# chlhnu/DOT-SOCP

Measured on AMD Instinct MI355X. Metric: ADMM iters/sec on NxNxT dot2d staggered grid at 1/2/4/8 MI355X, higher is better.
Workload: dtype f64

## Files before the change

dot-socp_amd/capi.py:

```python
import ctypes
import os

import numpy as np

_HERE = os.path.dirname(os.path.abspath(__file__))
LIB_PATH = os.path.join(_HERE, "lib", "libdotsocp.so")

i64 = ctypes.c_longlong
dbl = ctypes.c_double
vp = ctypes.c_void_p


class DotsocpError(RuntimeError):
    def __init__(self, code, msg):
        super().__init__(f"libdotsocp error {code}: {msg}")
        self.code = code


class Problem(ctypes.Structure):
    _fields_ = [("dim", ctypes.c_int), ("weighted", ctypes.c_int),
                ("ny", i64), ("nx", i64), ("nt", i64),
                ("D", dbl), ("E", dbl), ("cScale", dbl), ("dScale", dbl),
                ("normc", dbl), ("normd", dbl)]

# ... 30 lines not shown
    "dotsocp_bfd_conj1d": (ctypes.c_int, [vp, vp, i64, i64, dbl]),
    "dotsocp_oper_poisson": (ctypes.c_int, [vp, vp, i64, i64, i64, dbl]),
    "dotsocp_dctn": (ctypes.c_int, [vp, i64, i64, i64, ctypes.c_int]),
    "dotsocp_proj_soc_dev": (ctypes.c_int, [vp, vp, i64, i64, vp]),
    "dotsocp_bfd_dev": (ctypes.c_int, [vp, vp, i64, i64, i64, dbl, dbl, vp]),
    "dotsocp_bfd_conj_dev": (ctypes.c_int, [vp, vp, i64, i64, i64, dbl, vp]),
    "dotsocp_create": (vp, [ctypes.POINTER(Problem), ctypes.c_int, ctypes.c_int]),
    "dotsocp_create_multi": (vp, [ctypes.POINTER(Problem), ctypes.c_int, ctypes.c_int]),
    "dotsocp_destroy": (None, [vp]),
    "dotsocp_rccl_unique_id": (ctypes.c_int, [vp]),
    "dotsocp_attach_rccl": (ctypes.c_int, [vp, vp, ctypes.c_int, ctypes.c_int]),
    "dotsocp_slab_range": (ctypes.c_int, [i64, ctypes.c_int, ctypes.c_int, ctypes.POINTER(i64), ctypes.POINTER(i64)]),
    "dotsocp_field_len": (i64, [ctypes.POINTER(Problem), ctypes.c_int]),
    "dotsocp_dct_algorithm": (ctypes.c_int, [i64]),
    "dotsocp_tsolve_tri_safe": (ctypes.c_int, [i64, i64, i64]),
    "dotsocp_cone_writes_beta": (ctypes.c_int, [i64, dbl, i64, ctypes.c_int, ctypes.c_int, ctypes.c_int, dbl, dbl]),
    "dotsocp_rescale_due": (ctypes.c_int, [i64, ctypes.c_int, dbl, dbl]),
    "dotsocp_qcone_form": (ctypes.c_int, [i64, dbl, i64, ctypes.c_int, ctypes.c_int, ctypes.c_int, ctypes.c_int, dbl, dbl]),
    "dotsocp_release_cache": (i64, []),
    "dotsocp_upload": (ctypes.c_int, [vp, ctypes.c_int, vp]),
    "dotsocp_upload_layers": (ctypes.c_int, [vp, ctypes.c_int, vp, i64, i64]),
    "dotsocp_download": (ctypes.c_int, [vp, ctypes.c_int, vp]),
    "dotsocp_begin": (ctypes.c_int, [vp, ctypes.POINTER(Opts)]),
    "dotsocp_begin_method": (ctypes.c_int, [vp, ctypes.POINTER(Opts), ctypes.c_int, ctypes.POINTER(AccOpts)]),
    "dotsocp_run": (ctypes.c_int, [vp, i64, ctypes.POINTER(i64)]),
    "dotsocp_recover_outputs": (ctypes.c_int, [vp, vp, vp, vp, vp, vp, vp, vp, vp]),
    "dotsocp_jump_next_level": (ctypes.c_int, [vp, vp]),
    "dotsocp_finish": (ctypes.c_int, [vp, ctypes.POINTER(Result)]),
    "dotsocp_get_history": (ctypes.c_int, [vp, vp, vp, vp, vp]),
    "dotsocp_set_profiling": (ctypes.c_int, [vp, ctypes.c_int]),
# ... 76 lines not shown
```

dot-socp_amd/csrc/capi.hip:

```cpp
#include <cstring>
#include <new>

#include "comm.h"
#include "solver.h"

using namespace dotsocp;

namespace dotsocp {
extern thread_local std::string g_last_error;
int dotsocp_slab_range_impl(i64 nt, int world, int rank, i64 *t0, i64 *t1);
}

struct dotsocp_ctx {
    Solver s;
};

static int require_device() {
    int n = 0;
    if (hipGetDeviceCount(&n) != hipSuccess || n <= 0) {
        set_error("no HIP device available (libdotsocp has no CPU fallback)");
        return DOTSOCP_ENODEVICE;
    }
    return 0;
}
// ... 178 lines not shown
    DS_CHECK(pl.make(ny, nx, nt));
    const double pi = 3.14159265358979323846;
    auto table = [&](DevBuf &d, i64 m) -> int {
        std::vector<double> t((size_t)m);
        for (i64 k = 0; k < m; ++k) t[k] = (2.0 * (double)(m - 1) * (double)(m - 1)) * (1.0 - cos(pi * (double)k / (double)m));
        DS_CHECK(d.alloc(m));
        DS_HIP(hipMemcpy(d.p, t.data(), sizeof(double) * m, hipMemcpyHostToDevice));
        return 0;
    };
    DS_CHECK(table(cy, ny));
    DS_CHECK(table(cx, nx));
    DS_CHECK(table(ct, nt));
    DS_HIP(hipMemcpy(da.p, rhs, sizeof(double) * n, hipMemcpyHostToDevice));
    Grid g;
    g.set(ny, nx, nt, 0, nt);
    DS_CHECK(launch_dct_axis(pl.py, da.p, db.p, ny, nx, nt, 0, 0, nullptr));
    DS_CHECK(launch_dct_axis(pl.px, db.p, da.p, ny, nx, nt, 1, 0, nullptr));
    DS_CHECK(launch_poisson_t_single(pl.pt, g, kernelScale, cy.p, cx.p, ct.p, da.p, db.p, 0, nullptr, tsolve_tri_allowed()));
    DS_CHECK(launch_dct_axis(pl.px, da.p, db.p, ny, nx, nt, 1, 1, nullptr));
    DS_CHECK(launch_dct_axis(pl.py, db.p, da.p, ny, nx, nt, 0, 1, nullptr));
    DS_HIP(hipDeviceSynchronize());
    DS_HIP(hipMemcpy(res, da.p, sizeof(double) * n, hipMemcpyDeviceToHost));
    return 0;
}

dotsocp_ctx *dotsocp_create(const dotsocp_problem *prob, int device, int nslabs) {
    dotsocp_ctx *c = new (std::nothrow) dotsocp_ctx();
    if (!c) { set_error("out of host memory"); return nullptr; }
    if (c->s.init(prob, device, nslabs) != 0) {
        delete c;
        return nullptr;
    }
    return c;
}

// ... 26 lines not shown
}

int dotsocp_attach_rccl(dotsocp_ctx *ctx, const unsigned char id[128], int rank, int world) {
    if (!ctx) { set_error("ctx is NULL"); return DOTSOCP_EINVAL; }
    return ctx->s.attach_rccl(id, rank, world);
}

#define CTX_OR_FAIL()                                      \
    do {                                                   \
        if (!ctx) { set_error("ctx is NULL"); return DOTSOCP_EINVAL; } \
        (void)hipGetLastError();    \
    } while (0)

int dotsocp_dct_algorithm(dotsocp_i64 n) { return dct_choose_algorithm(n); }
int dotsocp_tsolve_tri_safe(dotsocp_i64 ny, dotsocp_i64 nx, dotsocp_i64 nt) { return tsolve_tri_safe(ny, nx, nt) ? 1 : 0; }

int dotsocp_cone_writes_beta(dotsocp_i64 it, double last_sigma_it, dotsocp_i64 maxit, int check_step_by_step,
                             int last_of_run, int rescale, double maxFeas, double relGap) {
    return cone_writes_beta(it, last_sigma_it, maxit, check_step_by_step != 0, last_of_run != 0, rescale, maxFeas, relGap) ? 1 : 0;
}
int dotsocp_rescale_due(dotsocp_i64 it, int rescale, double maxFeas, double relGap) {
    return rescale_due(it, rescale, maxFeas, relGap) ? 1 : 0;
}
int dotsocp_qcone_form(dotsocp_i64 it, double last_sigma_it, dotsocp_i64 maxit, int check_step_by_step, int last_of_run,
                       int next_last_of_run, int rescale, double maxFeas, double relGap) {
    return qcone_form(it, last_sigma_it, maxit, check_step_by_step != 0, last_of_run != 0, next_last_of_run != 0, rescale,
                      maxFeas, relGap);
}

dotsocp_i64 dotsocp_field_len(const dotsocp_problem *p, int field) {
// ... 94 lines not shown
```

dot-socp_amd/csrc/dct.hip:

```cpp
#include "cdft.h"
#include "dct_families.h"
#include "fft_lds.h"
#include "kernels.h"
#include "pfa.h"

#include <cstdlib>
#include <cstring>

namespace dotsocp {

#define CDFT_DEFAULT_MIN 500

int dct_choose_algorithm(i64 n) {
    static const bool pfa_on = !(getenv("DOTSOCP_PFA") && atoi(getenv("DOTSOCP_PFA")) == 0);
    static const bool cdft_on = !(getenv("DOTSOCP_CDFT") && atoi(getenv("DOTSOCP_CDFT")) == 0);
    static const i64 nb = [] {
        const char *e = getenv("DOTSOCP_CDFT_MIN");
        const i64 v = e ? atoll(e) : CDFT_DEFAULT_MIN;
        return v < 48 ? (i64)48 : v;
    }();
    if (n <= 1) return DCT_ALG_NONE;
    if ((n & (n - 1)) == 0) return DCT_ALG_FFT;
    if (pfa_supported(n)) return pfa_on ? DCT_ALG_PFA : DCT_ALG_DENSE;
    if (cdft_on && n == 257) return DCT_ALG_RADER;
// ... 164 lines not shown
    return !(e && strcmp(e, "dct") == 0);
}

int launch_poisson_t_single(const DctPlan *pt, const Grid &g, double kscale, const double *cy, const double *cx,
                            const double *ct, double *p, double *p2, i64 pitch0, hipStream_t st, bool allow_tri) {
    const i64 ny = g.ny, nx = g.nx, nt = g.nt;
    if (allow_tri && tsolve_tri_preferred(nt, dct_plan_is_pow2(pt), g.plane) && tsolve_tri_safe(ny, nx, nt))
        return launch_tsolve_tri(g, nt, kscale, cy, cx, p, st);
    if (dct_plan_has_tsolve(pt))
        return launch_dct_t_solve(pt, p, p, ny, ny * nx, 0, ny * nx, nt, kscale, cy, cx, ct, st, pitch0);
    DS_CHECK(launch_dct_axis(pt, p, p2, ny, nx, nt, 2, 0, st, pitch0));
    DS_CHECK(launch_spectral_divide(p2, ny, nt, 0, nx, kscale, cy, cx, ct, st, pitch0));
    return launch_dct_axis(pt, p2, p, ny, nx, nt, 2, 1, st, pitch0);
}

}
```

dot-socp_amd/csrc/dct_families.h:

```cpp
#pragma once
#include "common.h"

namespace dotsocp {

struct LineMap;
struct Pow2Plan;
struct DensePlan;

#define DCT_THREADS 256

Pow2Plan *pow2_plan_create(i64 n);
void pow2_plan_destroy(Pow2Plan *p);
int pow2_launch_axis0(const Pow2Plan *p, const double *src, double *dst, const LineMap &map, int inverse, hipStream_t st);
int pow2_launch_strided(const Pow2Plan *p, const double *src, double *dst, const LineMap &map, int inverse, hipStream_t st);
int pow2_launch_tsolve(const Pow2Plan *p, const double *src, double *dst, i64 ny, i64 nplane, i64 line0, i64 nl,
                       double kscale, const double *cy, const double *cx, const double *ct, hipStream_t st, i64 pitch0);

DensePlan *dense_plan_create(i64 n);
void dense_plan_destroy(DensePlan *p);
int dense_launch(const DensePlan *p, const double *src, double *dst, const LineMap &map, bool axis0, int inverse,
                 hipStream_t st);

}
```

dot-socp_amd/csrc/dct_pow2.hip:

```cpp
#include "dct_families.h"
#include "device_utils.h"
#include "fft_lds.h"
#include "kernels.h"

#include <cmath>
#include <cstdint>
#include <cstdlib>
#include <type_traits>
#include <utility>
#include <vector>

namespace dotsocp {

struct Pow2Plan {
    i64 n;
    int lg;
    double2 *tw;
    double2 *ww;
};

Pow2Plan *pow2_plan_create(i64 n) {
    Pow2Plan *p = new Pow2Plan();
    p->n = n;
    p->lg = 0;
// ... 556 lines not shown
                Bv = make_double2(p0.y, p1.y);
            } else {
                const double2 v0 = r[padi(bitrev(j0, LG))], v1 = r[padi(bitrev(n - 1 - j0, LG))];
                Av = make_double2(v0.x, v1.x);
                Bv = make_double2(v0.y, v1.y);
            }
            *(double2 *)(out + (2 * rr) * ls + 2 * j0) = Av;
            *(double2 *)(out + (2 * rr + 1) * ls + 2 * j0) = Bv;
        }
        if (tile + stride < nTiles) asm volatile("s_waitcnt vmcnt(%0)" ::"i"(PIPE_NS) : "memory");
        lds_barrier();
        if (tile + 2 * stride < nTiles) dma(tile + 2 * stride, b);
    }
}

template <int MODE , int LG>
__global__ void __launch_bounds__(PIPE_THREADS) k_dct_strided_pipe(const double *__restrict__ src, double *__restrict__ dst,
                                                                    LineMap map, int nTiles, const double2 *__restrict__ tw,
                                                                    const double2 *__restrict__ ww) {
    extern __shared__ double2 lds[];
    constexpr int n = 1 << LG;
    constexpr int lrows = PIPE_LG_CPLX - LG;
    constexpr int NP = 1 << lrows;
    constexpr int BUF = 1 << PIPE_LG_CPLX;
    constexpr bool BIG = LG > 10;
    constexpr int NTW = BIG ? (n >> 2) : (n >> 1), NWW = BIG ? (n >> 1) + 1 : n;
    double2 *twS = lds + 2 * BUF, *wwS = twS + NTW;
    const int tid = threadIdx.x, lane = tid & 63;
    const int wave = __builtin_amdgcn_readfirstlane(tid >> 6);
    for (int i = tid; i < NTW; i += PIPE_THREADS) twS[i] = tw[i];
// ... 429 lines not shown
        for_const<0, 1>(inverse ? 1 : 0, [&](auto i) {
            DS_KLAUNCH(k_dct_axis0_wg<decltype(i)::value != 0>, dim3(wblocks), dim3(DCT_WG_THREADS), lds, st, src, dst,
                       map.nLines, map.outerStride, lg, lrows, tw, ww);
        });
        DS_HIP(hipGetLastError());
        return 0;
    }
    for_const<0, 1>(inverse ? 1 : 0, [&](auto i) {
        DS_KLAUNCH(k_dct_axis0<decltype(i)::value != 0>, dim3(blocks), dim3(DCT_THREADS), lds, st, src, dst, map.nLines,
                   map.outerStride, lg, lrw, tw, ww);
    });
    DS_HIP(hipGetLastError());
    return 0;
}

}
```

dot-socp_amd/csrc/kernels.h:

```cpp
#pragma once
#include "common.h"
#include "defer.h"

namespace dotsocp {

struct LoopCoef {
    double s;
    double sf;
    double dF;
    double at, ax, ay;
    double tau;
    double c1, c2;
    double dinv1, dinv2;
};

enum {
    S_Q2 = 0, S_Z2, S_APHI2, S_ALPHA2, S_BETA2, S_FBBETA2, S_PRIM1, S_PRIM2, S_DUAL1, S_DUAL2,
    S_COMPLEM, S_DOTCOMP, S_RHO2, S_RHOFQ2, S_MRHOB, S_M2, S_RHOB2, S_QALPHA, S_CPHI, S_PHI2,
    S_COUNT
};

struct KktCoef {
    double sigma;
    double kappa;
// ... 153 lines not shown
    int world;
    i64 cut[DS_MAX_WORLD + 1];
};
int launch_pencil_pack(bool pack, const PencilCuts &pc, i64 plane, i64 ntl, double *slab, double *stage, hipStream_t st);

#define TRI_EXTRA 256
int launch_tri_local(const Grid &g, i64 nt, double kscale, const double *cy, const double *cx, const PencilCuts &pc,
                     const double *r, double *send, hipStream_t st);
int launch_tri_reduced(const Grid &g, i64 nt, double kscale, const double *cy, const double *cx, const PencilCuts &pc,
                       int rank, i64 l0, i64 nl, const i64 *slab_n, const double *recv, double *back, double *zero_work,
                       hipStream_t st, const double *own_recv = nullptr, double *own_back = nullptr);
int launch_tri_final(const Grid &g, i64 nt, double kscale, const double *cy, const double *cx, const PencilCuts &pc,
                     const double *back, double *x, hipStream_t st);
bool tsolve_tri_supported(i64 nt);
bool tsolve_tri_preferred(i64 nt, bool pow2, i64 plane);
bool tsolve_tri_safe(i64 ny, i64 nx, i64 nt);
int launch_tsolve_tri(const Grid &g, i64 nt, double kscale, const double *cy, const double *cx, double *x, hipStream_t st);
struct GatherMsgs {
    const double *src[DS_MAX_WORLD];
    double *dst[DS_MAX_WORLD];
    i64 count[DS_MAX_WORLD];
    int n;
};
int launch_gather_msgs(const GatherMsgs &m, hipStream_t st);

#define KKT_SLICES 64
struct KktWork {
    double *partials;
    i64 maxBlocks;
    double *sums;
// ... 26 lines not shown
void dct_plan_destroy(DctPlan *p);
int launch_dct_axis(const DctPlan *p, const double *src, double *dst, i64 n0, i64 n1, i64 n2, int axis,
                    int inverse, hipStream_t st, i64 pitch0 = 0);
bool dct_plan_is_pow2(const DctPlan *p);
bool dct_plan_has_tsolve(const DctPlan *p);
int launch_dct_t_solve(const DctPlan *p, const double *src, double *dst, i64 ny, i64 nplane, i64 line0, i64 nl,
                       i64 nt, double kscale, const double *cy, const double *cx, const double *ct, hipStream_t st,
                       i64 pitch0 = 0);
int launch_spectral_divide_pencil(double *data, i64 ny, i64 line0, i64 nl, i64 nt, double kscale, const double *cy,
                                  const double *cx, const double *ct, hipStream_t st);
int launch_spectral_divide(double *data, i64 ny, i64 nt, i64 x0, i64 nxl, double kscale, const double *cy,
                           const double *cx, const double *ct, hipStream_t st, i64 pitch0 = 0);
bool tsolve_tri_allowed();
int launch_poisson_t_single(const DctPlan *pt, const Grid &g, double kscale, const double *cy, const double *cx,
                            const double *ct, double *p, double *p2, i64 pitch0, hipStream_t st, bool allow_tri);

}
```

dot-socp_amd/csrc/solver.hip:

```cpp
#include "solver.h"

#include <algorithm>
#include <cmath>
#include <cstring>

#include "comm.h"

namespace dotsocp {

void Solver::update_coef() {
    lc.s = E / D;
    lc.sf = edge_factor(lc.s);
    lc.dF = E / dScale;
    const double ht = 1.0 / (double)(nt - 1);
    lc.at = D * (1.0 / ht);
    lc.ax = (nx > 1) ? D * (1.0 / (1.0 / (double)(nx - 1))) : 0.0;
    lc.ay = (ny > 1) ? D * (1.0 / (1.0 / (double)(ny - 1))) : 0.0;
    lc.tau = opts.tau;
    const double tmp = (E / D) * (E / D);
    if (prob.weighted) { lc.c1 = 2.0 * tmp; lc.c2 = tmp; }
    else { lc.c1 = 1.0 + 2.0 * tmp; lc.c2 = 1.0 + tmp; }
    lc.dinv1 = 1.0 / lc.c1;
    lc.dinv2 = 1.0 / lc.c2;
}
// ... 159 lines not shown
    if (canary_enabled() && getenv("DOTSOCP_CANARY_SELFTEST")) {
        Slab &s0 = slabs[0];
        DS_CHECK(use(s0));
        const double v = 1.0;
        DS_HIP(ds_memcpy_async(s0.c + s0.g.Nphi, &v, sizeof v, hipMemcpyHostToDevice, s0.st));
        DS_HIP(ds_stream_synchronize(s0.st));
    }
    begun = true;
    elapsed_prev = 0.0;
    elapsed_agreed = 0.0;
    t_begin = std::chrono::steady_clock::now();
    return 0;
}

int Solver::poisson_all(const PhiHooks *hooks) {
    const i64 plane = slabs[0].g.plane;
    const bool tp2 = dct_plan_has_tsolve(devres[0]->pt);
    FOR_SLABS(s) {
        const Grid &g = s.g;
        DS_CHECK(launch_dct_axis(s.res->py, s.w0, s.w1, g.ny, g.nx, g.ntl, 0, 0, s.st, g.py));
        DS_CHECK(launch_dct_axis(s.res->px, s.w1, s.w0, g.ny, g.nx, g.ntl, 1, 0, s.st, g.py));
    }
    bool tri = multi() && tri_tsolve && world <= DS_MAX_WORLD;
    for (auto &s : slabs) tri = tri && s.g.ntl <= TRI_EXTRA;
    if (tri) {
        DS_CHECK(poisson_t_tridiag(hooks));
    } else {
    if (hooks && hooks->fill) {
        prof_end(PH_POISSON);
        DS_CHECK(hooks->fill());
        prof_begin(PH_POISSON);
    }
    if (hooks && hooks->behind) DS_CHECK(hooks->behind());
    if (multi()) {
        prof_begin(PH_TRANSPOSE);
        DS_CHECK(transpose(true));
        prof_end(PH_TRANSPOSE);
    }
    FOR_SLABS(s) {
        double *p = multi() ? s.pencil : s.w0;
        double *p2 = multi() ? s.pencil2 : s.w1;
        if (!multi()) {
            DS_CHECK(launch_poisson_t_single(s.res->pt, s.g, D * D, s.res->cy, s.res->cx, s.res->ct, p, p2, s.g.py, s.st, tri_tsolve));
        } else if (tp2) {
            DS_CHECK(launch_dct_t_solve(s.res->pt, p, p, s.g.py, plane, s.l0, s.nl, nt, D * D, s.res->cy, s.res->cx, s.res->ct, s.st));
        } else {
            DS_CHECK(launch_dct_axis(s.res->pt, p, p2, s.nl, 1, nt, 2, 0, s.st));
            DS_CHECK(launch_spectral_divide_pencil(p2, s.g.py, s.l0, s.nl, nt, D * D, s.res->cy, s.res->cx, s.res->ct, s.st));
            DS_CHECK(launch_dct_axis(s.res->pt, p2, p, s.nl, 1, nt, 2, 1, s.st));
        }
    }
    if (multi()) {
        prof_begin(PH_TRANSPOSE);
        DS_CHECK(transpose(false));
        prof_end(PH_TRANSPOSE);
    }
    }
    FOR_SLABS(s) {
        const Grid &g = s.g;
        DS_CHECK(launch_dct_axis(s.res->px, s.w0, s.w1, g.ny, g.nx, g.ntl, 1, 1, s.st, g.py));
        DS_CHECK(launch_dct_axis(s.res->py, s.w1, s.phi, g.ny, g.nx, g.ntl, 0, 1, s.st, g.py));
    }
    return 0;
}

int Solver::poisson_phi() {
    if (begun) { set_error("poisson_phi() must precede begin()"); return DOTSOCP_ESTATE; }
    cur_dev = -1;
    DS_CHECK(use_dev(device));
    DS_CHECK(ensure_alloc());
    D = prob.D;
// ... 730 lines not shown
```

dot-socp_amd/csrc/tri.hip:

```cpp
#include "device_utils.h"
#include "kernels.h"

#include <cmath>
#include <cstdint>
#include <cstdlib>
#include <mutex>

namespace dotsocp {

struct TriGeom {
    i64 ny, plane, ntl;
    int first, last;
    double beta;
    double kscale;
    const double *cy, *cx;
    PencilCuts pc;
};

__device__ __forceinline__ double tri_aprime(const TriGeom &g, i64 m) { return (g.cy[m % g.ny] + g.cx[m / g.ny]) / g.beta; }

__device__ __forceinline__ int tri_owner(const PencilCuts &pc, i64 m, i64 plane) {
    int j = (int)((m * pc.world) / plane);
    while (j > 0 && m < pc.cut[j]) --j;
    while (j < pc.world - 1 && m >= pc.cut[j + 1]) ++j;
    return j;
}

__device__ __forceinline__ i64 tri_msg_off(const PencilCuts &pc, int j) { return 2 * pc.cut[j] + (i64)TRI_EXTRA * j; }

struct TriCoef {
    double rho, rho2, r, r2, n0d;
};
__device__ __forceinline__ TriCoef tri_coef(double ap) {
    TriCoef c;
    const double s = sqrt(ap * (1.0 + 0.25 * ap));
    const double rm1 = 0.5 * ap + s;
    c.r = 1.0 + rm1;
    c.rho = 1.0 / c.r;
    c.rho2 = c.rho * c.rho;
    c.r2 = c.r * c.r;
    c.n0d = (rm1 * c.rho) * (1.0 + c.rho);
    return c;
}
__device__ __forceinline__ double tri_n0(const TriCoef &c, bool bnd) { return bnd ? 1.0 + c.rho : c.n0d; }
__device__ __forceinline__ double tri_div(double x, double n) {
    double r = __builtin_amdgcn_rcp(n);
    double e = __builtin_fma(-n, r, 1.0);
    r = __builtin_fma(r, e, r);
    e = __builtin_fma(-n, r, 1.0);
    r = __builtin_fma(r, e, r);
    const double q = x * r;
    return __builtin_fma(__builtin_fma(-n, q, x), r, q);
}
struct TriEnds {
    double N0, N1, Nn, s, pe;
};
__device__ __forceinline__ TriEnds tri_ends(const TriCoef &c, bool bnd, int n, double rn1) {
    TriEnds e;
    e.s = bnd ? 1.0 : -1.0;
    e.pe = bnd ? c.rho : c.rho2;
    e.N0 = tri_n0(c, bnd);
    e.N1 = (n == 1) ? e.N0 : 1.0 + e.s * ((rn1 * rn1) * e.pe);
    e.Nn = c.n0d + c.rho2 * e.N1;
    return e;
}
__device__ __forceinline__ double tri_powi(double x, int k) {
    double r = 1.0;
    while (k > 0) {
        if (k & 1) r *= x;
        x *= x;
        k >>= 1;
    }
    return r;
}
__device__ __forceinline__ double tri_last(const TriCoef &c, double D, double N1, double Nn, bool bnd) {
    return bnd ? tri_div(D, c.r * Nn - N1) : tri_div(c.rho * D, Nn);
}
#define TRI_PW_SAFE 0x1p-500
struct TriSpike {
    double vf, vl, wf, wl;
};
__device__ __forceinline__ TriSpike tri_spike(const TriCoef &c, int n, bool first, bool last) {
    const double rn1 = tri_powi(c.rho, n - 1);
    const TriEnds f = tri_ends(c, first, n, rn1), b = tri_ends(c, last, n, rn1);
    TriSpike k;
    if (last) {
        const double den = c.r * f.Nn - f.N1;
        k.vl = tri_div(rn1 * f.N0, den);
        k.wl = tri_div(f.N1, den);
    } else {
        k.vl = tri_div((rn1 * c.rho) * f.N0, f.Nn);
        k.wl = tri_div(c.rho * f.N1, f.Nn);
    }
// ... 598 lines not shown

bool tsolve_tri_safe(i64 ny, i64 nx, i64 nt) {
    if (!tsolve_tri_supported(nt)) return false;
    const int nsub = tsolve_nsub(nt);
    const double n = (double)((nt + nsub - 1) / nsub);
    const double ap = 4.0 * ((double)(ny - 1) * (double)(ny - 1) + (double)(nx - 1) * (double)(nx - 1)) /
                      ((double)(nt - 1) * (double)(nt - 1));
    const double r = 1.0 + 0.5 * ap + sqrt(ap * (1.0 + 0.25 * ap));
    return (n - 1.0) * log2(r) <= 500.0;
}

static bool tsolve_pipe_on() {
    const char *pe = getenv("DOTSOCP_TS_PIPE");
    return !(pe && atoi(pe) == 0);
}
static bool tsolve_pipe_fits(i64 nt, i64 plane) {
    return nt > 64 && nt <= 136 && (plane + 63) / 64 >= 16 * (i64)tri_device_cus() && (plane % 2) == 0;
}
bool tsolve_tri_preferred(i64 nt, bool pow2, i64 plane) {
    if (!tsolve_tri_supported(nt)) return false;
    return !pow2 || (tsolve_pipe_on() && tsolve_pipe_fits(nt, plane));
}

int launch_tsolve_tri(const Grid &g, i64 nt, double kscale, const double *cy, const double *cx, double *x, hipStream_t st) {
    PencilCuts pc{};
    pc.world = 1;
    pc.cut[0] = 0;
    pc.cut[1] = g.plane;
    const TriGeom t = make_geom(g, nt, kscale, cy, cx, pc);
    const dim3 grid((unsigned)((g.plane + 63) / 64));
    const int nTiles = (int)((g.plane + 63) / 64);
// ... 58 lines not shown
```

include/dotsocp.h:

```cpp
#ifndef DOTSOCP_H
#define DOTSOCP_H

#ifdef __cplusplus
extern "C" {
#endif

typedef long long dotsocp_i64;

enum {
    DOTSOCP_OK = 0,
    DOTSOCP_EINVAL = -1,
    DOTSOCP_ENODEVICE = -2,
    DOTSOCP_EHIP = -3,
    DOTSOCP_ESTATE = -4,
    DOTSOCP_ECOMM = -5
};

const char *dotsocp_last_error(void);
const char *dotsocp_version(void);
int dotsocp_device_count(void);
dotsocp_i64 dotsocp_release_cache(void);


int dotsocp_proj_soc(double *out, const double *in, dotsocp_i64 M, dotsocp_i64 K);
// ... 78 lines not shown
dotsocp_ctx *dotsocp_create(const dotsocp_problem *prob, int device, int nslabs);
dotsocp_ctx *dotsocp_create_multi(const dotsocp_problem *prob, int first_device, int ngpu);
void dotsocp_destroy(dotsocp_ctx *ctx);

int dotsocp_rccl_unique_id(unsigned char id[128]);
int dotsocp_attach_rccl(dotsocp_ctx *ctx, const unsigned char id[128], int rank, int world);

int dotsocp_slab_range(dotsocp_i64 nt, int world, int rank, dotsocp_i64 *t0, dotsocp_i64 *t1);

dotsocp_i64 dotsocp_field_len(const dotsocp_problem *prob, int field);

int dotsocp_dct_algorithm(dotsocp_i64 n);

int dotsocp_tsolve_tri_safe(dotsocp_i64 ny, dotsocp_i64 nx, dotsocp_i64 nt);

int dotsocp_cone_writes_beta(dotsocp_i64 it, double last_sigma_it, dotsocp_i64 maxit, int check_step_by_step,
                             int last_of_run, int rescale, double maxFeas, double relGap);
int dotsocp_rescale_due(dotsocp_i64 it, int rescale, double maxFeas, double relGap);
int dotsocp_qcone_form(dotsocp_i64 it, double last_sigma_it, dotsocp_i64 maxit, int check_step_by_step, int last_of_run,
                       int next_last_of_run, int rescale, double maxFeas, double relGap);

int dotsocp_upload(dotsocp_ctx *ctx, int field, const double *host);
int dotsocp_download(dotsocp_ctx *ctx, int field, double *host);
int dotsocp_upload_layers(dotsocp_ctx *ctx, int field, const double *host, dotsocp_i64 t0, dotsocp_i64 n);

int dotsocp_begin(dotsocp_ctx *ctx, const dotsocp_opts *opts);
int dotsocp_begin_method(dotsocp_ctx *ctx, const dotsocp_opts *opts, int method, const dotsocp_acc_opts *acc);
int dotsocp_run(dotsocp_ctx *ctx, dotsocp_i64 n_iters, dotsocp_i64 *done);
int dotsocp_finish(dotsocp_ctx *ctx, dotsocp_result *res);

// ... 21 lines not shown
```

Baseline: 98.96.

## Fold the temporal tridiagonal solve into the y-axis DCT pass of the Poisson solve

Adds a marching kernel that performs the y-axis DCT and the t-direction tridiagonal solve in one pass over time tiles, so the single-device Poisson solve goes from five passes to four. This removes one full read and write of the volume and a separate tsolve launch. The fold is gated by a shape heuristic (power-of-two ny of at least 128, enough x-columns to fill the CUs, nt within the pipe range) and an environment override. It adds a serial per-mode march over time inside the kernel, which can limit parallelism. The single- and multi-slab Poisson paths are also refactored onto a shared launch_poisson_single helper.

After: 102.4, median of 6. +3.4%, better.

```diff
diff --git a/dot-socp_amd/capi.py b/dot-socp_amd/capi.py
--- a/dot-socp_amd/capi.py
+++ b/dot-socp_amd/capi.py
@@ -68,6 +68,7 @@
     "dotsocp_field_len": (i64, [ctypes.POINTER(Problem), ctypes.c_int]),
     "dotsocp_dct_algorithm": (ctypes.c_int, [i64]),
     "dotsocp_tsolve_tri_safe": (ctypes.c_int, [i64, i64, i64]),
+    "dotsocp_poisson_fold_form": (ctypes.c_int, [i64, i64, i64]),
     "dotsocp_cone_writes_beta": (ctypes.c_int, [i64, dbl, i64, ctypes.c_int, ctypes.c_int, ctypes.c_int, dbl, dbl]),
     "dotsocp_rescale_due": (ctypes.c_int, [i64, ctypes.c_int, dbl, dbl]),
     "dotsocp_qcone_form": (ctypes.c_int, [i64, dbl, i64, ctypes.c_int, ctypes.c_int, ctypes.c_int, ctypes.c_int, dbl, dbl]),
diff --git a/dot-socp_amd/csrc/capi.hip b/dot-socp_amd/csrc/capi.hip
--- a/dot-socp_amd/csrc/capi.hip
+++ b/dot-socp_amd/csrc/capi.hip
@@ -216,11 +216,8 @@
     DS_HIP(hipMemcpy(da.p, rhs, sizeof(double) * n, hipMemcpyHostToDevice));
     Grid g;
     g.set(ny, nx, nt, 0, nt);
-    DS_CHECK(launch_dct_axis(pl.py, da.p, db.p, ny, nx, nt, 0, 0, nullptr));
-    DS_CHECK(launch_dct_axis(pl.px, db.p, da.p, ny, nx, nt, 1, 0, nullptr));
-    DS_CHECK(launch_poisson_t_single(pl.pt, g, kernelScale, cy.p, cx.p, ct.p, da.p, db.p, 0, nullptr, tsolve_tri_allowed()));
-    DS_CHECK(launch_dct_axis(pl.px, da.p, db.p, ny, nx, nt, 1, 1, nullptr));
-    DS_CHECK(launch_dct_axis(pl.py, db.p, da.p, ny, nx, nt, 0, 1, nullptr));
+    DS_CHECK(launch_poisson_single(pl.py, pl.px, pl.pt, g, kernelScale, cy.p, cx.p, ct.p, da.p, db.p, da.p, nullptr,
+                                   tsolve_tri_allowed()));
     DS_HIP(hipDeviceSynchronize());
     DS_HIP(hipMemcpy(res, da.p, sizeof(double) * n, hipMemcpyDeviceToHost));
     return 0;
@@ -277,6 +274,9 @@
 
 int dotsocp_dct_algorithm(dotsocp_i64 n) { return dct_choose_algorithm(n); }
 int dotsocp_tsolve_tri_safe(dotsocp_i64 ny, dotsocp_i64 nx, dotsocp_i64 nt) { return tsolve_tri_safe(ny, nx, nt) ? 1 : 0; }
+int dotsocp_poisson_fold_form(dotsocp_i64 ny, dotsocp_i64 nx, dotsocp_i64 nt) {
+    return poisson_fold_form(ny, nx, nt, tsolve_tri_allowed());
+}
 
 int dotsocp_cone_writes_beta(dotsocp_i64 it, double last_sigma_it, dotsocp_i64 maxit, int check_step_by_step,
                              int last_of_run, int rescale, double maxFeas, double relGap) {
diff --git a/dot-socp_amd/csrc/dct.hip b/dot-socp_amd/csrc/dct.hip
--- a/dot-socp_amd/csrc/dct.hip
+++ b/dot-socp_amd/csrc/dct.hip
@@ -202,4 +202,38 @@
     return launch_dct_axis(pt, p2, p, ny, nx, nt, 2, 1, st, pitch0);
 }
 
-}
+
+int poisson_fold_form(i64 ny, i64 nx, i64 nt, bool allow_tri) {
+    const char *e = getenv("DOTSOCP_POISSON_FOLD");
+    const int sw = (e && *e) ? (atoi(e) != 0 ? 1 : 0) : -1;
+    if (sw == 0 || !allow_tri || !pow2_march_shape_ok(ny, nx, nt)) return 0;
+    if (sw == 1) return 1;
+    const i64 plane = ny * nx;
+    const i64 cols = 1024 / ny;
+    return tsolve_tri_preferred(nt, (nt & (nt - 1)) == 0, plane) && tsolve_tri_safe(ny, nx, nt) && tsolve_pipe_fits(nt, plane) &&
+           ny >= 128 && (nx + cols - 1) / cols >= (i64)pow2_march_workgroups();
+}
+
+int launch_poisson_single(const DctPlan *py, const DctPlan *px, const DctPlan *pt, const Grid &g, double kscale,
+                          const double *cy, const double *cx, const double *ct, double *w0, double *w1, double *out,
+                          hipStream_t st, bool allow_tri, const std::function<int()> *between) {
+    const i64 ny = g.ny, nx = g.nx, nt = g.nt;
+    const bool fold = dct_plan_is_pow2(py) && poisson_fold_form(ny, nx, nt, allow_tri) != 0;
+    if (fold) {
+        DS_CHECK(launch_dct_axis(px, w0, w1, ny, nx, nt, 1, 0, st, g.py));
+        DS_CHECK(pow2_launch_axis0_march(py->pow2, w1, w0, nx, nt, g.py, g.plane, 0, kscale, cy, cx, st));
+    } else {
+        DS_CHECK(launch_dct_axis(py, w0, w1, ny, nx, nt, 0, 0, st, g.py));
+        DS_CHECK(launch_dct_axis(px, w1, w0, ny, nx, nt, 1, 0, st, g.py));
+    }
+    if (between && *between) DS_CHECK((*between)());
+    if (fold) {
+        DS_CHECK(pow2_launch_axis0_march(py->pow2, w0, w1, nx, nt, g.py, g.plane, 1, kscale, cy, cx, st));
+        return launch_dct_axis(px, w1, out, ny, nx, nt, 1, 1, st, g.py);
+    }
+    DS_CHECK(launch_poisson_t_single(pt, g, kscale, cy, cx, ct, w0, w1, g.py, st, allow_tri));
+    DS_CHECK(launch_dct_axis(px, w0, w1, ny, nx, nt, 1, 1, st, g.py));
+    return launch_dct_axis(py, w1, out, ny, nx, nt, 0, 1, st, g.py);
+}
+
+}
diff --git a/dot-socp_amd/csrc/dct_families.h b/dot-socp_amd/csrc/dct_families.h
--- a/dot-socp_amd/csrc/dct_families.h
+++ b/dot-socp_amd/csrc/dct_families.h
@@ -15,6 +15,10 @@
 int pow2_launch_strided(const Pow2Plan *p, const double *src, double *dst, const LineMap &map, int inverse, hipStream_t st);
 int pow2_launch_tsolve(const Pow2Plan *p, const double *src, double *dst, i64 ny, i64 nplane, i64 line0, i64 nl,
                        double kscale, const double *cy, const double *cx, const double *ct, hipStream_t st, i64 pitch0);
+bool pow2_march_shape_ok(i64 ny, i64 nx, i64 nt);
+int pow2_march_workgroups();
+int pow2_launch_axis0_march(const Pow2Plan *p, const double *src, double *dst, i64 nx, i64 nt, i64 ls, i64 plane, int inverse,
+                            double kscale, const double *cy, const double *cx, hipStream_t st);
 
 DensePlan *dense_plan_create(i64 n);
 void dense_plan_destroy(DensePlan *p);
diff --git a/dot-socp_amd/csrc/dct_pow2.hip b/dot-socp_amd/csrc/dct_pow2.hip
--- a/dot-socp_amd/csrc/dct_pow2.hip
+++ b/dot-socp_amd/csrc/dct_pow2.hip
@@ -2,6 +2,7 @@
 #include "device_utils.h"
 #include "fft_lds.h"
 #include "kernels.h"
+#include "tri_coef.h"
 
 #include <cmath>
 #include <cstdint>
@@ -594,6 +595,207 @@
     }
 }
 
+#define MARCH_ROWS 8
+struct MarchArgs {
+    int nx, nt;
+    i64 plane;
+    double sc, beta;
+    const double *cy, *cx;
+};
+
+template <bool INVERSE, int LG>
+__global__ void __launch_bounds__(PIPE_THREADS) k_dct_axis0_march(const double *__restrict__ src, double *__restrict__ dst,
+                                                                   int nItems, i64 ls ,
+                                                                   MarchArgs ma, const double2 *__restrict__ tw,
+                                                                   const double2 *__restrict__ ww) {
+    extern __shared__ double2 lds[];
+    constexpr int n = 1 << LG, lh = LG - 1;
+    constexpr int LPT = (2 << PIPE_LG_CPLX) / n;
+    constexpr int NXC = LPT / MARCH_ROWS;
+    constexpr int PPL = n / 128;
+    constexpr int RS = n + 1;
+    constexpr int lrows = PIPE_LG_CPLX - LG;
+    constexpr int BUF = RS << lrows;
+    static_assert(LG >= 7 && LG <= 10 && PIPE_IT * 2 == MARCH_ROWS, "a thread holds all rows of its two modes");
+    double2 *twS = lds + 2 * BUF, *wwS = twS + (n >> 1);
+    double *zcol = (double *)(wwS + n);
+    const int tid = threadIdx.x, lane = tid & 63;
+    const int wave = __builtin_amdgcn_readfirstlane(tid >> 6);
+    for (int i = tid; i < (n >> 1); i += PIPE_THREADS) twS[i] = tw[i];
+    for (int i = tid; i < n; i += PIPE_THREADS) wwS[i] = ww[i];
+    const int j0 = tid & ((1 << lh) - 1);
+    const int hcol = wave >> (lh - 6);
+    double cyv[2] = {ma.cy[2 * j0], ma.cy[2 * j0 + 1]};
+    const int nt = ma.nt;
+    if (INVERSE && blockIdx.x == 0) {
+        for (int t = tid; t < nt; t += PIPE_THREADS) zcol[t] = src[(i64)t * ma.plane];
+        __syncthreads();
+        if (tid == 0) {
+            double sum = 0.0;
+            for (int t = 0; t < nt; ++t) sum += zcol[t];
+            const double gbar = sum / (double)nt;
+            double xm = 0.0, xc = 0.0, acc = 0.0;
+            for (int t = 0; t < nt; ++t) {
+                const double gt = zcol[t] - gbar;
+                zcol[t] = xc;
+                acc += xc;
+                const double xn = (t == 0) ? xc - gt : 2.0 * xc - xm - gt;
+                xm = xc;
+                xc = xn;
+            }
+            const double shift = ma.beta * gbar - acc / (double)nt;
+            for (int t = 0; t < nt; ++t) zcol[t] += shift;
+        }
+    }
+    asm volatile("s_waitcnt vmcnt(0)" : "+v"(cyv[0]), "+v"(cyv[1])::"memory");
+    const unsigned ldsBase = (unsigned)(uintptr_t)lds;
+    const int tpi = nt / MARCH_ROWS;
+    const int w = blockIdx.x, stride = gridDim.x;
+    const int nq = (w < nItems) ? ((nItems - 1 - w) / stride + 1) * tpi : 0;
+    auto tile_item = [&](int q) { return w + (q / tpi) * stride; };
+    auto tile_t0 = [&](int q) { return INVERSE ? nt - MARCH_ROWS * (q % tpi + 1) : MARCH_ROWS * (q % tpi); };
+    auto column = [&](int item, int h) { const int x = item * NXC + h; return x < ma.nx ? x : ma.nx - 1; };
+    auto dma = [&](int q, int b) {
+        const int item = tile_item(q), t0 = tile_t0(q);
+        const char *g = (const char *)src + lane * 16;
+        const unsigned l0 = ldsBase + (unsigned)b * (unsigned)(BUF * 16) + (unsigned)(wave * PIPE_ND) * 1024u;
+#pragma unroll
+        for (int i = 0; i < PIPE_ND; ++i) {
+            const int piece = wave * PIPE_ND + i, l = piece / PPL;
+            const int rr = l >> 1, t = t0 + 2 * (rr / NXC) + (l & 1);
+            const i64 off = (i64)column(item, rr % NXC) * ls + (i64)t * ma.plane;
+            glds16(g + off * 8 + (piece % PPL) * 1024, l0 + (unsigned)i * 1024u);
+        }
+    };
+    if (0 < nq) dma(0, 0);
+    if (1 < nq) dma(1, 1);
+    if (1 < nq) asm volatile("s_waitcnt vmcnt(%0)" ::"i"(PIPE_ND) : "memory");
+    else asm volatile("s_waitcnt vmcnt(0)" ::: "memory");
+    lds_barrier();
+    auto item_row = [&](int u) { return (tid + u * PIPE_THREADS) >> lh; };
+    double rho[2], H[2], G[2], pw[2];
+    double rr_[2], Nt1[2], xn[2];
+    int ts[2];
+    bool zero = false;
+    auto item_begin = [&](int item, double2 *last) {
+        const int x = column(item, hcol);
+        const double ex = sload_f64(ma.cx + x);
+        zero = (x == 0 && j0 == 0);
+#pragma unroll
+        for (int m = 0; m < 2; ++m) {
+            const TriCoef c = tri_coef((zero && m == 0) ? 1.0 : (cyv[m] + ex) / ma.beta);
+            rho[m] = c.rho;
+            if (!INVERSE) {
+                H[m] = 0.0; G[m] = 0.0; pw[m] = 1.0;
+            } else {
+                double p = 1.0, ps = 1.0;
+                int tsafe = 0;
+#pragma unroll 1
+                for (int t = 0; t < nt; ++t) {
+                    if (p >= TRI_PW_SAFE) { tsafe = t; ps = p; }
+                    if (t + 1 < nt) p *= c.rho;
+                }
+                const TriEnds f = tri_ends(c, true, nt, p);
+                rr_[m] = c.r; Nt1[m] = f.N1; pw[m] = ps; ts[m] = tsafe;
+                double &v = m == 0 ? last->x : last->y;
+                v = xn[m] = tri_last(c, v, f.N1, f.Nn, true);
+            }
+        }
+    };
+    auto march = [&](int m, int t, double v, bool bottom = false) -> double {
+        if (!INVERSE) {
+            const double g = v * ma.sc;
+            const double D = tri_fwd_row(rho[m], rho[m], g, pw[m], H[m], G[m]);
+            pw[m] *= rho[m];
+            return (zero && m == 0) ? g : D;
+        } else {
+            pw[m] = (t < ts[m]) ? pw[m] * rr_[m] : pw[m];
+            double Nt = (t > ts[m]) ? 1.0 : tri_nt(rho[m], pw[m]);
+            Nt = bottom ? 1.0 + rho[m] : Nt;
+            xn[m] = tri_back_row(rho[m], v, Nt, xn[m], Nt1[m]);
+            Nt1[m] = Nt;
+            return xn[m];
+        }
+    };
+    for (int q = 0; q < nq; ++q) {
+        const int b = q & 1;
+        double2 *buf = lds + b * BUF;
+        const int item = tile_item(q), t0 = tile_t0(q);
+        const bool first_tile = (q % tpi == 0);
+        {
+            const double *raw = (const double *)buf;
+            double2 A[PIPE_IT], B[PIPE_IT];
+#pragma unroll
+            for (int u = 0; u < PIPE_IT; ++u) {
+                const int rr = item_row(u);
+                A[u] = *(const double2 *)(raw + (2 * rr) * n + 2 * j0);
+                B[u] = *(const double2 *)(raw + (2 * rr + 1) * n + 2 * j0);
+            }
+            if (INVERSE) {
+                constexpr int UL = PIPE_IT - 1;
+                if (first_tile) {
+                    item_begin(item, &B[UL]);
+                } else {
+                    B[UL].x = march(0, t0 + 2 * UL + 1, B[UL].x);
+                    B[UL].y = march(1, t0 + 2 * UL + 1, B[UL].y);
+                }
+                A[UL].x = march(0, t0 + 2 * UL, A[UL].x);
+                A[UL].y = march(1, t0 + 2 * UL, A[UL].y);
+#pragma unroll
+                for (int u = UL - 1; u >= 0; --u) {
+                    B[u].x = march(0, t0 + 2 * u + 1, B[u].x);
+                    B[u].y = march(1, t0 + 2 * u + 1, B[u].y);
+                    A[u].x = march(0, t0 + 2 * u, A[u].x, u == 0 && t0 == 0);
+                    A[u].y = march(1, t0 + 2 * u, A[u].y, u == 0 && t0 == 0);
+                }
+                if (zero) {
+#pragma unroll
+                    for (int u = 0; u < PIPE_IT; ++u) {
+                        A[u].x = zcol[t0 + 2 * u];
+                        B[u].x = zcol[t0 + 2 * u + 1];
+                    }
+                }
+            }
+            lds_barrier();
+#pragma unroll
+            for (int u = 0; u < PIPE_IT; ++u) {
+                double2 *r = buf + item_row(u) * RS;
+                if (!INVERSE) {
+                    r[padi(j0)] = make_double2(A[u].x, B[u].x);
+                    r[padi(n - 1 - j0)] = make_double2(A[u].y, B[u].y);
+                } else {
+                    r[padi(2 * j0)] = make_double2(A[u].x, B[u].x);
+                    r[padi(2 * j0 + 1)] = make_double2(A[u].y, B[u].y);
+                }
+            }
+        }
+        lds_barrier();
+        if (INVERSE) idct_combine_wg<true>(buf, lrows, LG, RS, tid, PIPE_THREADS, (const double2 *)wwS);
+        fft_rows_pipe<LG, lrows, PIPE_THREADS, RS>(buf, tid, (const double2 *)twS);
+        if (!INVERSE && first_tile) item_begin(item, nullptr);
+        double *out = dst + (i64)column(item, hcol) * ls + (i64)t0 * ma.plane + 2 * j0;
+#pragma unroll
+        for (int u = 0; u < PIPE_IT; ++u) {
+            const double2 *r = buf + item_row(u) * RS;
+            double2 Av, Bv;
+            if (!INVERSE) {
+                const double2 p0 = dct_post(r, 2 * j0, n, LG, (const double2 *)wwS), p1 = dct_post(r, 2 * j0 + 1, n, LG, (const double2 *)wwS);
+                Av = make_double2(march(0, t0 + 2 * u, p0.x), march(1, t0 + 2 * u, p1.x));
+                Bv = make_double2(march(0, t0 + 2 * u + 1, p0.y), march(1, t0 + 2 * u + 1, p1.y));
+            } else {
+                const double2 v0 = r[padi(bitrev(j0, LG))], v1 = r[padi(bitrev(n - 1 - j0, LG))];
+                Av = make_double2(v0.x, v1.x);
+                Bv = make_double2(v0.y, v1.y);
+            }
+            *(double2 *)(out + (i64)(2 * u) * ma.plane) = Av;
+            *(double2 *)(out + (i64)(2 * u + 1) * ma.plane) = Bv;
+        }
+        if (q + 1 < nq) asm volatile("s_waitcnt vmcnt(%0)" ::"i"(PIPE_NS) : "memory");
+        lds_barrier();
+        if (q + 2 < nq) dma(q + 2, b);
+    }
+}
+
 template <int MODE , int LG>
 __global__ void __launch_bounds__(PIPE_THREADS) k_dct_strided_pipe(const double *__restrict__ src, double *__restrict__ dst,
                                                                     LineMap map, int nTiles, const double2 *__restrict__ tw,
@@ -1053,4 +1255,45 @@
     return 0;
 }
 
-}
+int pow2_march_workgroups() { return device_cus(); }
+
+bool pow2_march_shape_ok(i64 ny, i64 nx, i64 nt) {
+    if (!dct_pipe_enabled() || ny < (1 << PIPE_LG_MIN) || ny > 1024 || (ny & (ny - 1))) return false;
+    return nx >= 1 && nx < (1ll << 28) && nt >= MARCH_ROWS && nt % MARCH_ROWS == 0 && tsolve_tri_supported(nt);
+}
+
+int pow2_launch_axis0_march(const Pow2Plan *p, const double *src, double *dst, i64 nx, i64 nt, i64 ls, i64 plane, int inverse,
+                            double kscale, const double *cy, const double *cx, hipStream_t st) {
+    const i64 n = p->n;
+    const int lg = p->lg;
+    if (!pow2_march_shape_ok(n, nx, nt) || ls < n || (ls % 2) || (plane % 2) || plane < ls * nx ||
+        (((uintptr_t)src | (uintptr_t)dst) % 16) || src == dst) {
+        set_error("marching y pass: unsupported shape %lld x %lld x %lld (pitch %lld)", (long long)n, (long long)nx, (long long)nt,
+                  (long long)ls);
+        return DOTSOCP_EINVAL;
+    }
+    static unsigned long long done_march = 0;
+    if (DeviceOnce once_(done_march); once_)
+        for_const<PIPE_LG_MIN, 10>(ALL_CONST, [](auto c) {
+            allow_big_lds(k_dct_axis0_march<false, decltype(c)::value>);
+            allow_big_lds(k_dct_axis0_march<true, decltype(c)::value>);
+        });
+    const i64 cols = 1024 / n;
+    const int nItems = (int)((nx + cols - 1) / cols);
+    const double beta = (double)(nt - 1) * (double)(nt - 1);
+    const MarchArgs ma{(int)nx, (int)nt, plane, 1.0 / (kscale * beta), beta, cy, cx};
+    const size_t ldsPipe = (2 * (((size_t)n + 1) << (PIPE_LG_CPLX - lg)) + (size_t)(n >> 1) + (size_t)n) * sizeof(double2) +
+                           (size_t)nt * sizeof(double);
+    if (ldsPipe > DCT_LDS_MAX) { set_error("marching y pass: nt = %lld does not fit the LDS", (long long)nt); return DOTSOCP_EINVAL; }
+    const double2 *tw = p->tw, *ww = p->ww;
+    for_const<PIPE_LG_MIN, 10>(lg, [&](auto c) {
+        for_const<0, 1>(inverse ? 1 : 0, [&](auto i) {
+            DS_KLAUNCH((k_dct_axis0_march<decltype(i)::value != 0, decltype(c)::value>), dim3((unsigned)device_cus()),
+                       dim3(PIPE_THREADS), ldsPipe, st, src, dst, nItems, ls, ma, tw, ww);
+        });
+    });
+    DS_HIP(hipGetLastError());
+    return 0;
+}
+
+}
diff --git a/dot-socp_amd/csrc/kernels.h b/dot-socp_amd/csrc/kernels.h
--- a/dot-socp_amd/csrc/kernels.h
+++ b/dot-socp_amd/csrc/kernels.h
@@ -1,4 +1,5 @@
 #pragma once
+#include <functional>
 #include "common.h"
 #include "defer.h"
 
@@ -191,6 +192,7 @@
                      const double *back, double *x, hipStream_t st);
 bool tsolve_tri_supported(i64 nt);
 bool tsolve_tri_preferred(i64 nt, bool pow2, i64 plane);
+bool tsolve_pipe_fits(i64 nt, i64 plane);
 bool tsolve_tri_safe(i64 ny, i64 nx, i64 nt);
 int launch_tsolve_tri(const Grid &g, i64 nt, double kscale, const double *cy, const double *cx, double *x, hipStream_t st);
 struct GatherMsgs {
@@ -247,5 +249,9 @@
 bool tsolve_tri_allowed();
 int launch_poisson_t_single(const DctPlan *pt, const Grid &g, double kscale, const double *cy, const double *cx,
                             const double *ct, double *p, double *p2, i64 pitch0, hipStream_t st, bool allow_tri);
+int poisson_fold_form(i64 ny, i64 nx, i64 nt, bool allow_tri);
+int launch_poisson_single(const DctPlan *py, const DctPlan *px, const DctPlan *pt, const Grid &g, double kscale,
+                          const double *cy, const double *cx, const double *ct, double *w0, double *w1, double *out,
+                          hipStream_t st, bool allow_tri, const std::function<int()> *between = nullptr);
 
 }
diff --git a/dot-socp_amd/csrc/solver.hip b/dot-socp_amd/csrc/solver.hip
--- a/dot-socp_amd/csrc/solver.hip
+++ b/dot-socp_amd/csrc/solver.hip
@@ -197,6 +197,21 @@
 }
 
 int Solver::poisson_all(const PhiHooks *hooks) {
+    if (!multi()) {
+        Slab &s = slabs[0];
+        DS_CHECK(use(s));
+        const std::function<int()> between = [&]() -> int {
+            if (hooks && hooks->fill) {
+                prof_end(PH_POISSON);
+                DS_CHECK(hooks->fill());
+                prof_begin(PH_POISSON);
+            }
+            if (hooks && hooks->behind) DS_CHECK(hooks->behind());
+            return 0;
+        };
+        return launch_poisson_single(s.res->py, s.res->px, s.res->pt, s.g, D * D, s.res->cy, s.res->cx, s.res->ct, s.w0, s.w1,
+                                     s.phi, s.st, tri_tsolve, &between);
+    }
     const i64 plane = slabs[0].g.plane;
     const bool tp2 = dct_plan_has_tsolve(devres[0]->pt);
     FOR_SLABS(s) {
@@ -204,40 +219,33 @@
         DS_CHECK(launch_dct_axis(s.res->py, s.w0, s.w1, g.ny, g.nx, g.ntl, 0, 0, s.st, g.py));
         DS_CHECK(launch_dct_axis(s.res->px, s.w1, s.w0, g.ny, g.nx, g.ntl, 1, 0, s.st, g.py));
     }
-    bool tri = multi() && tri_tsolve && world <= DS_MAX_WORLD;
+    bool tri = tri_tsolve && world <= DS_MAX_WORLD;
     for (auto &s : slabs) tri = tri && s.g.ntl <= TRI_EXTRA;
     if (tri) {
         DS_CHECK(poisson_t_tridiag(hooks));
     } else {
-    if (hooks && hooks->fill) {
-        prof_end(PH_POISSON);
-        DS_CHECK(hooks->fill());
-        prof_begin(PH_POISSON);
-    }
-    if (hooks && hooks->behind) DS_CHECK(hooks->behind());
-    if (multi()) {
+        if (hooks && hooks->fill) {
+            prof_end(PH_POISSON);
+            DS_CHECK(hooks->fill());
+            prof_begin(PH_POISSON);
+        }
+        if (hooks && hooks->behind) DS_CHECK(hooks->behind());
         prof_begin(PH_TRANSPOSE);
         DS_CHECK(transpose(true));
         prof_end(PH_TRANSPOSE);
-    }
-    FOR_SLABS(s) {
-        double *p = multi() ? s.pencil : s.w0;
-        double *p2 = multi() ? s.pencil2 : s.w1;
-        if (!multi()) {
-            DS_CHECK(launch_poisson_t_single(s.res->pt, s.g, D * D, s.res->cy, s.res->cx, s.res->ct, p, p2, s.g.py, s.st, tri_tsolve));
-        } else if (tp2) {
-            DS_CHECK(launch_dct_t_solve(s.res->pt, p, p, s.g.py, plane, s.l0, s.nl, nt, D * D, s.res->cy, s.res->cx, s.res->ct, s.st));
-        } else {
-            DS_CHECK(launch_dct_axis(s.res->pt, p, p2, s.nl, 1, nt, 2, 0, s.st));
-            DS_CHECK(launch_spectral_divide_pencil(p2, s.g.py, s.l0, s.nl, nt, D * D, s.res->cy, s.res->cx, s.res->ct, s.st));
-            DS_CHECK(launch_dct_axis(s.res->pt, p2, p, s.nl, 1, nt, 2, 1, s.st));
-        }
-    }
-    if (multi()) {
+        FOR_SLABS(s) {
+            double *p = s.pencil, *p2 = s.pencil2;
+            if (tp2) {
+                DS_CHECK(launch_dct_t_solve(s.res->pt, p, p, s.g.py, plane, s.l0, s.nl, nt, D * D, s.res->cy, s.res->cx, s.res->ct, s.st));
+            } else {
+                DS_CHECK(launch_dct_axis(s.res->pt, p, p2, s.nl, 1, nt, 2, 0, s.st));
+                DS_CHECK(launch_spectral_divide_pencil(p2, s.g.py, s.l0, s.nl, nt, D * D, s.res->cy, s.res->cx, s.res->ct, s.st));
+                DS_CHECK(launch_dct_axis(s.res->pt, p2, p, s.nl, 1, nt, 2, 1, s.st));
+            }
+        }
         prof_begin(PH_TRANSPOSE);
         DS_CHECK(transpose(false));
         prof_end(PH_TRANSPOSE);
-    }
     }
     FOR_SLABS(s) {
         const Grid &g = s.g;
diff --git a/dot-socp_amd/csrc/tri.hip b/dot-socp_amd/csrc/tri.hip
--- a/dot-socp_amd/csrc/tri.hip
+++ b/dot-socp_amd/csrc/tri.hip
@@ -1,5 +1,6 @@
 #include "device_utils.h"
 #include "kernels.h"
+#include "tri_coef.h"
 
 #include <cmath>
 #include <cstdint>
@@ -28,55 +29,6 @@
 
 __device__ __forceinline__ i64 tri_msg_off(const PencilCuts &pc, int j) { return 2 * pc.cut[j] + (i64)TRI_EXTRA * j; }
 
-struct TriCoef {
-    double rho, rho2, r, r2, n0d;
-};
-__device__ __forceinline__ TriCoef tri_coef(double ap) {
-    TriCoef c;
-    const double s = sqrt(ap * (1.0 + 0.25 * ap));
-    const double rm1 = 0.5 * ap + s;
-    c.r = 1.0 + rm1;
-    c.rho = 1.0 / c.r;
-    c.rho2 = c.rho * c.rho;
-    c.r2 = c.r * c.r;
-    c.n0d = (rm1 * c.rho) * (1.0 + c.rho);
-    return c;
-}
-__device__ __forceinline__ double tri_n0(const TriCoef &c, bool bnd) { return bnd ? 1.0 + c.rho : c.n0d; }
-__device__ __forceinline__ double tri_div(double x, double n) {
-    double r = __builtin_amdgcn_rcp(n);
-    double e = __builtin_fma(-n, r, 1.0);
-    r = __builtin_fma(r, e, r);
-    e = __builtin_fma(-n, r, 1.0);
-    r = __builtin_fma(r, e, r);
-    const double q = x * r;
-    return __builtin_fma(__builtin_fma(-n, q, x), r, q);
-}
-struct TriEnds {
-    double N0, N1, Nn, s, pe;
-};
-__device__ __forceinline__ TriEnds tri_ends(const TriCoef &c, bool bnd, int n, double rn1) {
-    TriEnds e;
-    e.s = bnd ? 1.0 : -1.0;
-    e.pe = bnd ? c.rho : c.rho2;
-    e.N0 = tri_n0(c, bnd);
-    e.N1 = (n == 1) ? e.N0 : 1.0 + e.s * ((rn1 * rn1) * e.pe);
-    e.Nn = c.n0d + c.rho2 * e.N1;
-    return e;
-}
-__device__ __forceinline__ double tri_powi(double x, int k) {
-    double r = 1.0;
-    while (k > 0) {
-        if (k & 1) r *= x;
-        x *= x;
-        k >>= 1;
-    }
-    return r;
-}
-__device__ __forceinline__ double tri_last(const TriCoef &c, double D, double N1, double Nn, bool bnd) {
-    return bnd ? tri_div(D, c.r * Nn - N1) : tri_div(c.rho * D, Nn);
-}
-#define TRI_PW_SAFE 0x1p-500
 struct TriSpike {
     double vf, vl, wf, wl;
 };
@@ -705,7 +657,7 @@
     const char *pe = getenv("DOTSOCP_TS_PIPE");
     return !(pe && atoi(pe) == 0);
 }
-static bool tsolve_pipe_fits(i64 nt, i64 plane) {
+bool tsolve_pipe_fits(i64 nt, i64 plane) {
     return nt > 64 && nt <= 136 && (plane + 63) / 64 >= 16 * (i64)tri_device_cus() && (plane % 2) == 0;
 }
 bool tsolve_tri_preferred(i64 nt, bool pow2, i64 plane) {
diff --git a/dot-socp_amd/csrc/tri_coef.h b/dot-socp_amd/csrc/tri_coef.h
--- /dev/null
+++ b/dot-socp_amd/csrc/tri_coef.h
@@ -0,0 +1,76 @@
+#pragma once
+#include "common.h"
+
+namespace dotsocp {
+
+struct TriCoef {
+    double rho, rho2, r, r2, n0d;
+};
+__device__ __forceinline__ TriCoef tri_coef(double ap) {
+#pragma clang fp contract(off)
+    TriCoef c;
+    const double s = sqrt(ap * (1.0 + 0.25 * ap));
+    const double rm1 = 0.5 * ap + s;
+    c.r = 1.0 + rm1;
+    c.rho = 1.0 / c.r;
+    c.rho2 = c.rho * c.rho;
+    c.r2 = c.r * c.r;
+    c.n0d = (rm1 * c.rho) * (1.0 + c.rho);
+    return c;
+}
+__device__ __forceinline__ double tri_n0(const TriCoef &c, bool bnd) { return bnd ? 1.0 + c.rho : c.n0d; }
+__device__ __forceinline__ double tri_div(double x, double n) {
+#pragma clang fp contract(off)
+    double r = __builtin_amdgcn_rcp(n);
+    double e = __builtin_fma(-n, r, 1.0);
+    r = __builtin_fma(r, e, r);
+    e = __builtin_fma(-n, r, 1.0);
+    r = __builtin_fma(r, e, r);
+    const double q = x * r;
+    return __builtin_fma(__builtin_fma(-n, q, x), r, q);
+}
+struct TriEnds {
+    double N0, N1, Nn, s, pe;
+};
+__device__ __forceinline__ TriEnds tri_ends(const TriCoef &c, bool bnd, int n, double rn1) {
+#pragma clang fp contract(off)
+    TriEnds e;
+    e.s = bnd ? 1.0 : -1.0;
+    e.pe = bnd ? c.rho : c.rho2;
+    e.N0 = tri_n0(c, bnd);
+    e.N1 = (n == 1) ? e.N0 : 1.0 + e.s * ((rn1 * rn1) * e.pe);
+    e.Nn = c.n0d + c.rho2 * e.N1;
+    return e;
+}
+__device__ __forceinline__ double tri_powi(double x, int k) {
+#pragma clang fp contract(off)
+    double r = 1.0;
+    while (k > 0) {
+        if (k & 1) r *= x;
+        x *= x;
+        k >>= 1;
+    }
+    return r;
+}
+__device__ __forceinline__ double tri_last(const TriCoef &c, double D, double N1, double Nn, bool bnd) {
+#pragma clang fp contract(off)
+    return bnd ? tri_div(D, c.r * Nn - N1) : tri_div(c.rho * D, Nn);
+}
+#define TRI_PW_SAFE 0x1p-500
+
+__device__ __forceinline__ double tri_fwd_row(double rho, double spe, double gt, double pw, double &H, double &G) {
+#pragma clang fp contract(off)
+    H = gt + rho * H;
+    G += pw * gt;
+    return H + (spe * pw) * G;
+}
+__device__ __forceinline__ double tri_nt(double spe, double pw) {
+#pragma clang fp contract(off)
+    return 1.0 + spe * (pw * pw);
+}
+__device__ __forceinline__ double tri_back_row(double rho, double Dt, double Nt, double xn, double Nt1) {
+#pragma clang fp contract(off)
+    return tri_div(rho * (Dt + Nt * xn), Nt1);
+}
+
+}
diff --git a/include/dotsocp.h b/include/dotsocp.h
--- a/include/dotsocp.h
+++ b/include/dotsocp.h
@@ -116,6 +116,8 @@
 
 int dotsocp_tsolve_tri_safe(dotsocp_i64 ny, dotsocp_i64 nx, dotsocp_i64 nt);
 
+int dotsocp_poisson_fold_form(dotsocp_i64 ny, dotsocp_i64 nx, dotsocp_i64 nt);
+
 int dotsocp_cone_writes_beta(dotsocp_i64 it, double last_sigma_it, dotsocp_i64 maxit, int check_step_by_step,
                              int last_of_run, int rescale, double maxFeas, double relGap);
 int dotsocp_rescale_due(dotsocp_i64 it, int rescale, double maxFeas, double relGap);
```
